# hassony2/homan

Hardware: AMD Instinct MI355X
Metric: optimisation iters/sec (30-frame 256^2 clip) (higher is better)
Workload: dtype f32

## Files before the change

### homan_amd/csrc/raster_api.hip

```cpp
#include "raster_ws.h"

RasterTune& hm_raster_tune()
{
    static thread_local RasterTune t = {0, 0, SWEEP_BLOCKS};
    return t;
}
int& hm_sweep_cap_override()
{
    static int cap = 0;
    return cap;
}

extern "C" {

size_t hm_sil_workspace_bytes(int B, int V, int F, int S)
{
    const size_t is = 2 * (size_t)S;
    size_t n = 256;
    n += al256((size_t)B * 16);
    n += al256((size_t)B * V * 3 * 4);
    n += al256((size_t)B * F * 9 * 4);
    n += al256((size_t)B * F * 8);
    n += al256((size_t)B * is * is * 4);
    n += al256((size_t)B * is * (is / 16) * 2);
    n += al256((size_t)B * S * S * 4);
    n += al256((size_t)B * (S / 8) * (S / 8) * 16);
    n += al256((size_t)B * is * is * 4);
    n += al256((size_t)B * is * (is / 16) * 4);
    n += al256((size_t)B * is * (is / 16) * 4);
    n += al256((size_t)B * F * 24 * 4);
    n += al256((size_t)B * F * 2);
    n += al256((size_t)B * SR_MAX * 8);
    n += al256((size_t)B * (S / 16) * (S / 16));
    n += al256((size_t)B * SR_MAX * F * 4);
    n += al256(4 * (size_t)B * is * (is / 64) * 16);
    n += al256((size_t)B * 2 * is * 16);
    n += al256(4 * (size_t)B * is * is * sizeof(SweepSrc));
    n += al256((size_t)B * F * sizeof(SweepFace));
    n += al256((size_t)B * F * 4) * 2;
    n += al256(sweep_ucap(B, F) * 4);
    n += al256(sweep_slot_cap(B, F) * 24);
    n += al256(ts_units(B, F, S) * 16);
    n += al256(ts_raster_units(B, S) * 4) * 3;
    return n;
}

int hm_tune_raster_lds_pad(int bytes)
{
    const int prev = hm_raster_tune().raster_lds_pad;
    if (bytes >= 0) hm_raster_tune().raster_lds_pad = bytes;
    return prev;
}
int hm_tune_raster_reorder(int enable)
{
    const int prev = hm_raster_tune().raster_reorder;
    if (enable >= 0) hm_raster_tune().raster_reorder = enable ? 1 : 0;
    return prev;
// ... 2 lines not shown
int hm_tune_sweep_blocks(int blocks)
{
    const int prev = hm_raster_tune().sweep_blocks;
    if (blocks > 0) hm_raster_tune().sweep_blocks = blocks;
    return prev;
}

int hm_sil_fwd_phase_clips(const float* verts, const int* faces, int faces_bstride, const float* K, int B, int V, int F, int S,
                           float orig_size, float znear, float zfar, const float* keep, const float* ref,
                           const float* keep_sum, float* pooled, float* loss_out, const int* work_order, float* pooled_depth,
                           float* alpha_full, int mask_shared, const float* rigid_rot6d, const float* rigid_trans,
                           const float* rigid_scale, int rigid_abs, int persistent_outputs, void* workspace, int clip_len,
                           int out_stride, float* cam_verts_out, int phases, hipStream_t stream)
{
    HM_CHECK_ARG(phases >= 1 && phases <= 3);
    HM_CHECK_ARG(verts && faces && K && pooled && workspace && HM_CLIP_LEN_OK(B, clip_len));
    if (clip_len == 0) clip_len = B;
    HM_CHECK_ARG(!rigid_rot6d || (rigid_trans && rigid_scale));
    HM_CHECK_ARG(B > 0 && V > 0 && F > 0 && S > 0);
    if (S % 16 != 0 || 2 * S > 8192 || 2L * F >= (1L << 30) || B >= 32768) return HM_ERR_UNSUPPORTED;
    HM_CHECK_ARG(faces_bstride == 0 || faces_bstride == 3 * F);
    SilWs w = carve(workspace, B, V, F, S);
    const int is = 2 * S;
    int* bins = is <= (SR_MAX == 64 ? 1024 : 0) ? w.bin_cnt : nullptr;
    HM_CHECK_ARG(!cam_verts_out || rigid_rot6d);
    if (phases & 1)
        hm_launch_setup_faces(w, verts, K, orig_size, faces, faces_bstride, B, V, F, is, bins, rigid_rot6d, rigid_trans, rigid_scale,
                              rigid_abs, clip_len, cam_verts_out, stream);
    if (!(phases & 2)) return hm_launch_status();
    const bool fused = keep && ref;
    const RasterTune& tune = hm_raster_tune();
    RasterFwdArgs a = {B, F, S, znear, zfar, pooled, keep, ref, fused, work_order, pooled_depth, bins, 1, persistent_outputs,
                       alpha_full, mask_shared, fused && (alpha_full || (mask_shared & 2)), tune.raster_reorder != 0,
                       tune.raster_lds_pad};
    hm_launch_raster_fwd(w, a, stream);
    if (fused && keep_sum && loss_out) hm_launch_sil_reduce(w, B, S, keep_sum, loss_out, nullptr, clip_len, out_stride, stream);
    return hm_launch_status();
}
int hm_sil_fwd_clips(const float* verts, const int* faces, int faces_bstride, const float* K, int B, int V, int F, int S,
                     float orig_size, float znear, float zfar, const float* keep, const float* ref,
                     const float* keep_sum, float* pooled, float* loss_out, const int* work_order, float* pooled_depth,
                     float* alpha_full, int mask_shared, const float* rigid_rot6d, const float* rigid_trans,
                     const float* rigid_scale, int rigid_abs, int persistent_outputs, void* workspace, int clip_len,
                     int out_stride, float* cam_verts_out, hipStream_t stream)
{
    return hm_sil_fwd_phase_clips(verts, faces, faces_bstride, K, B, V, F, S, orig_size, znear, zfar, keep, ref, keep_sum, pooled,
                                  loss_out, work_order, pooled_depth, alpha_full, mask_shared, rigid_rot6d, rigid_trans,
// ... 10 lines not shown
                            loss_out, work_order, pooled_depth, alpha_full, mask_shared, rigid_rot6d, rigid_trans,
                            rigid_scale, rigid_abs, persistent_outputs, workspace, 0, 0, nullptr, stream);
}

size_t hm_sil_render_bytes(void) { return sizeof(HmSilRender); }
int hm_sil_fwd_multi(const HmSilRender* renders, int n, int phases, hipStream_t stream)
{
    HM_CHECK_ARG(renders && n >= 1 && n <= HM_MAX_RENDERS && phases >= 1 && phases <= 3);
    SilWs ws[HM_MAX_RENDERS];
    SetupFacesArgs sa[HM_MAX_RENDERS];
    RasterFwdArgs ra[HM_MAX_RENDERS];
    const RasterTune& tune = hm_raster_tune();
    for (int g = 0; g < n; ++g) {
        const HmSilRender& r = renders[g];
        HM_CHECK_ARG(r.verts && r.faces && r.K && r.pooled && r.workspace && HM_CLIP_LEN_OK(r.B, r.clip_len));
        HM_CHECK_ARG(!r.rigid_rot6d || (r.rigid_trans && r.rigid_scale));
        HM_CHECK_ARG(r.B > 0 && r.V > 0 && r.F > 0 && r.S > 0 && (!r.keep == !r.ref));
        if (r.S % 16 != 0 || 2 * r.S > 8192 || 2L * r.F >= (1L << 30) || r.B >= 32768) return HM_ERR_UNSUPPORTED;
        HM_CHECK_ARG(r.faces_bstride == 0 || r.faces_bstride == 3 * r.F);
        HM_CHECK_ARG(!r.cam_verts_out || r.rigid_rot6d);
        for (int q = 0; q < g; ++q) HM_CHECK_ARG(renders[q].workspace != r.workspace);
        ws[g] = carve(r.workspace, r.B, r.V, r.F, r.S);
        const int is = 2 * r.S;
        int* bins = is <= (SR_MAX == 64 ? 1024 : 0) ? ws[g].bin_cnt : nullptr;
        const SetupFacesArgs s1 = {r.verts, r.K, r.orig_size, r.faces, r.faces_bstride, r.B, r.V, r.F, is, bins, r.rigid_rot6d,
                                   r.rigid_trans, r.rigid_scale, r.rigid_abs, r.clip_len ? r.clip_len : r.B, r.cam_verts_out};
        sa[g] = s1;
        const bool fused = r.keep && r.ref;
        const RasterFwdArgs r1 = {r.B, r.F, r.S, r.znear, r.zfar, r.pooled, r.keep, r.ref, fused, r.work_order, r.pooled_depth, bins, 1,
                                  r.persistent_outputs, nullptr, r.mask_shared & 1, false, tune.raster_reorder != 0, tune.raster_lds_pad};
        ra[g] = r1;
    }
    if (phases & 1) hm_launch_setup_faces_multi(ws, sa, n, stream);
    if (phases & 2) hm_launch_raster_fwd_multi(ws, ra, n, stream);
    return hm_launch_status();
}

int hm_sil_hint_near_winding(void* workspace, int winding, hipStream_t stream)
{
    HM_CHECK_ARG(workspace && (winding == 0 || winding == 1));
    return hipMemsetAsync((char*)workspace + 24 * 4, winding, 1, stream) == hipSuccess ? HM_OK : HM_ERR_LAUNCH;
}

int hm_sil_reduce_clips(int B, int V, int F, int S, const float* keep_sum, float* loss_out, float* frame_out,
                        void* workspace, int clip_len, int out_stride, hipStream_t stream)
{
    HM_CHECK_ARG(workspace && B > 0 && S > 0 && (frame_out || loss_out) && (!loss_out || keep_sum));
// ... 64 lines not shown
                        background, rgb, stream);
    return hm_launch_status();
}


int hm_bench_sil_kernels(const float* verts, const int* faces, const float* K, int B, int V, int F, int S,
                         const float* keep, const float* ref, const float* keep_sum, float* pooled, float* loss_out,
                         const int* work_order, const int* adj_off, const int* adj_items,
                         const float* upstream, float* grad_verts, void* workspace, int reps, float* avg_ms,
                         hipStream_t stream)
{
    HM_CHECK_ARG(verts && faces && K && keep && ref && keep_sum && pooled && loss_out && workspace && reps > 0 && avg_ms);
    HM_CHECK_ARG(adj_off && adj_items && upstream && grad_verts);
    int rc = hm_sil_fwd(verts, faces, 0, K, B, V, F, S, 1.0f, 0.1f, 100.0f, keep, ref, keep_sum, pooled, loss_out,
                        work_order, nullptr, nullptr, 0, nullptr, nullptr, nullptr, 0, 0, workspace, stream);
    if (rc != HM_OK) return rc;
    rc = hm_sil_bwd(verts, K, B, V, F, S, 1.0f, 1e-3f, 1, upstream, nullptr, keep_sum, adj_off, adj_items,
                    grad_verts, nullptr, workspace, 0, stream);
    if (rc != HM_OK) return rc;
    SilWs w = carve(workspace, B, V, F, S);
    hipEvent_t e0, e1;
    if (hipEventCreate(&e0) != hipSuccess || hipEventCreate(&e1) != hipSuccess) return HM_ERR_LAUNCH;
    float ms = 0.f;
    int* bins = 2 * S <= 1024 ? w.bin_cnt : nullptr;
    hm_launch_setup_faces(w, verts, K, 1.0f, faces, 0, B, V, F, 2 * S, bins, nullptr, nullptr, nullptr, 0, B, nullptr, stream);
    RasterFwdArgs a = {B, F, S, 0.1f, 100.0f, pooled, keep, ref, true, work_order, nullptr, bins, 0, 1, nullptr, 0, false, false, 0};
    (void)hipEventRecord(e0, stream);
    for (int i = 0; i < reps; ++i) hm_launch_raster_fwd(w, a, stream);
    (void)hipEventRecord(e1, stream);
    (void)hipEventSynchronize(e1);
    (void)hipEventElapsedTime(&ms, e0, e1);
    avg_ms[0] = ms / (float)reps;
    (void)hipMemsetAsync(w.bin_cnt, 0, (size_t)B * SR_MAX * 4, stream);
    (void)hipEventRecord(e0, stream);
    for (int i = 0; i < reps; ++i) hm_launch_sweep(w, B, F, S, 1e-3f, 0, stream);
    (void)hipEventRecord(e1, stream);
    (void)hipEventSynchronize(e1);
    (void)hipEventElapsedTime(&ms, e0, e1);
    avg_ms[1] = ms / (float)reps;
    (void)hipEventRecord(e0, stream);
    for (int i = 0; i < reps; ++i) hm_launch_lines(w, B, F, S, 1, upstream, keep_sum, B, stream);
    (void)hipEventRecord(e1, stream);
    (void)hipEventSynchronize(e1);
    (void)hipEventElapsedTime(&ms, e0, e1);
    avg_ms[2] = ms / (float)reps;
    (void)hipEventDestroy(e0);
    (void)hipEventDestroy(e1);
    return hm_launch_status();
}

size_t hm_sil_timestamps_bytes(int B, int V, int F, int S) { (void)V; return ts_units(B, F, S) * 16; }
int hm_sil_timestamps(void* workspace, int B, int V, int F, int S, int enable, hipStream_t stream)
{
    HM_CHECK_ARG(workspace && B > 0 && F > 0 && S > 0);
    SilWs w = carve(workspace, B, V, F, S);
    if (hipMemsetAsync((char*)workspace + 24 * 4 + 1, enable ? 1 : 0, 1, stream) != hipSuccess) return HM_ERR_LAUNCH;
// ... 31 lines not shown
    }
    free(t);
    return HM_OK;
}
int hm_debug_sweep_caps(int cap)
{
    const int prev = hm_sweep_cap_override();
    hm_sweep_cap_override() = cap > 0 ? cap : 0;
    return prev;
}

int hm_sil_read_idx_map(const void* workspace, int B, int V, int F, int S, int* out, hipStream_t stream)
{
    SilWs w = carve((void*)workspace, B, V, F, S);
    return hipMemcpyAsync(out, w.idx_map, (size_t)B * 4 * S * S * 4, hipMemcpyDeviceToDevice, stream) == hipSuccess
               ? HM_OK : HM_ERR_LAUNCH;
}
int hm_sil_read_boxes(const void* workspace, int B, int V, int F, int S, void* out, hipStream_t stream)
{
    SilWs w = carve((void*)workspace, B, V, F, S);
    return hipMemcpyAsync(out, w.boxes, (size_t)B * F * 8, hipMemcpyDeviceToDevice, stream) == hipSuccess ? HM_OK
                                                                                                         : HM_ERR_LAUNCH;
}
int hm_sil_read_faces9(const void* workspace, int B, int V, int F, int S, float* out, hipStream_t stream)
{
    SilWs w = carve((void*)workspace, B, V, F, S);
    return hipMemcpyAsync(out, w.faces9, (size_t)B * F * 9 * 4, hipMemcpyDeviceToDevice, stream) == hipSuccess
               ? HM_OK : HM_ERR_LAUNCH;
}
int hm_sil_invalidate_outputs(void* workspace, int B, int V, int F, int S, hipStream_t stream)
{
    HM_CHECK_ARG(workspace && B > 0 && S > 0);
    SilWs w = carve(workspace, B, V, F, S);
    return hipMemsetAsync(w.region_state, 0, (size_t)B * (S / 16) * (S / 16), stream) == hipSuccess ? HM_OK : HM_ERR_LAUNCH;
}
int hm_sil_read_parts(const void* workspace, int B, int V, int F, int S, double* out, hipStream_t stream)
{
    SilWs w = carve((void*)workspace, B, V, F, S);
    return hipMemcpyAsync(out, w.parts, (size_t)B * F * 6 * 8, hipMemcpyDeviceToDevice, stream) == hipSuccess
               ? HM_OK : HM_ERR_LAUNCH;
}
}
```

### homan_amd/csrc/raster_common.h

```cpp
#pragma once
#include "hm_common.h"
#include <type_traits>

#define HM_TILE 8
#define HM_STILE 16
#define RASTER_WAVES 4
#define STAGE_DW 20

typedef int hm_v2i __attribute__((ext_vector_type(2)));
typedef unsigned hm_v4u __attribute__((ext_vector_type(4)));
#ifndef RASTER_NT_STORES
#define RASTER_NT_STORES 0
#endif
__device__ __forceinline__ void hm_out_store(float* p, float v)
{
#if RASTER_NT_STORES
    __builtin_nontemporal_store(v, p);
#else
    *p = v;
#endif
}
__device__ __forceinline__ void hm_out_store2(int* p, int a, int b)
{
#if RASTER_NT_STORES
// ... 15 lines not shown

struct FaceBox {
    unsigned short x0m, y0, x1, y1;
};

__device__ __forceinline__ float topix(float v, int is)
{
    float a = v * (float)is;
    a = a + (float)is;
    a = a - 1.0f;
    return 0.5f * a;
}
__device__ __forceinline__ bool backside(const float* f)
{
    return (f[7] - f[1]) * (f[3] - f[0]) < (f[4] - f[1]) * (f[6] - f[0]);
}
__device__ __forceinline__ void wave_sync()
{
    __builtin_amdgcn_fence(__ATOMIC_ACQ_REL, "wavefront");
    __builtin_amdgcn_wave_barrier();
}

#define SR_MAX 64
__host__ __device__ __forceinline__ int hm_sr_shift(int is) { return is <= 512 ? 6 : 7; }

__device__ __forceinline__ int hm_wave_scan_incl(int v)
{
    v += __builtin_amdgcn_update_dpp(0, v, 0x111, 0xf, 0xf, false);
    v += __builtin_amdgcn_update_dpp(0, v, 0x112, 0xf, 0xf, false);
    v += __builtin_amdgcn_update_dpp(0, v, 0x114, 0xf, 0xf, false);
    v += __builtin_amdgcn_update_dpp(0, v, 0x118, 0xf, 0xf, false);
    v += __builtin_amdgcn_update_dpp(0, v, 0x142, 0xa, 0xf, false);
    v += __builtin_amdgcn_update_dpp(0, v, 0x143, 0xc, 0xf, false);
    return v;
}

__device__ __forceinline__ float rlane(float v, int l)
{
    return __builtin_bit_cast(float, __builtin_amdgcn_readlane(__builtin_bit_cast(int, v), l));
}

__device__ __forceinline__ unsigned spread8(unsigned x)
{
    x = (x | (x << 4)) & 0x0f0fu;
    x = (x | (x << 2)) & 0x3333u;
    x = (x | (x << 1)) & 0x5555u;
    return x;
// ... 125 lines not shown
```

### homan_amd/csrc/raster_fwd.hip

```cpp
#include "raster_ws.h"

#ifdef RASTER_TRACE
#define RASTER_TRACE_WGS 65536
__device__ unsigned g_raster_trace[RASTER_TRACE_WGS][9];
__device__ int g_raster_trace_F = 0, g_raster_trace_depth = -1;
#define RPH_MARK(k) do { if (tid == 0) { const unsigned long long t_ = wall_clock64(); rtr[k] += (unsigned)(t_ - rtr_t); rtr_t = t_; } } while (0)
#elif defined(RASTER_PHASES)
__device__ unsigned long long g_raster_ph[24];
#define RPH_MARK(k) do { if (tid == 0) { const unsigned long long t_ = clock64(); rph[k] += t_ - rph_t; rph_t = t_; } } while (0)
#else
#define RPH_MARK(k)
#endif
#ifndef CAND_CAP
#define CAND_CAP 512
#endif
#ifndef RB_PASS
#define RB_PASS 128
#endif
#ifndef HM_PRUNE
#define HM_PRUNE 1
#endif
#ifndef RASTER_WPE
#define RASTER_WPE 6
#endif
// ... 19 lines not shown
    __shared__ int wsum[RASTER_WAVES];
    __shared__ int cand_n[2];
    const int w = __builtin_amdgcn_readfirstlane((int)(threadIdx.x >> 6)), lane = threadIdx.x & 63, tid = threadIdx.x;
    const int is = 2 * S, tiles_x = S / HM_TILE, ntiles = tiles_x * tiles_x, regions_x = tiles_x / 2;
    const bool dyn = wo_dyn && hint[2] != 0u;
    const int wo = __builtin_amdgcn_readfirstlane(dyn ? wo_dyn[blk]
                                                     : work_order ? work_order[blk] : (int)(((blk % B) << 16) | (blk / B)));
    if (wo_dyn && !dyn && threadIdx.x == 0) wo_dyn[blk] = wo;
    const int region = wo & 0xffff, b = wo >> 16;
    const int rx = region % regions_x, ry = region / regions_x;
    const int tx = 2 * rx + (w & 1), ty = 2 * ry + (w >> 1);
    const int tile = ty * tiles_x + tx;

    const int gx0 = rx * 2 * HM_STILE, gx1 = gx0 + 2 * HM_STILE - 1;
    const int gy1 = is - 1 - ry * 2 * HM_STILE, gy0 = gy1 - (2 * HM_STILE - 1);
    const float gcx0 = (float)(2 * gx0 + 1 - is) / (float)is, gcx1 = (float)(2 * gx1 + 1 - is) / (float)is;
    const float gcy0 = (float)(2 * gy0 + 1 - is) / (float)is, gcy1 = (float)(2 * gy1 + 1 - is) / (float)is;
    const bool pow2 = (is & (is - 1)) == 0;
    const float inv_is = 1.0f / (float)is;
    const unsigned long long zb_empty = ((unsigned long long)__float_as_uint(zfar) << 32) | 0xffffffffull;

    int had_any = 0;
    const uint2* bx = reinterpret_cast<const uint2*>(boxes) + (long)b * F;
    const int nsx = (is + (1 << hm_sr_shift(is)) - 1) >> hm_sr_shift(is);
    const int sr = (gy0 >> hm_sr_shift(is)) * nsx + (gx0 >> hm_sr_shift(is));
    unsigned char* rstate = region_state + (long)b * regions_x * regions_x + region;
    const int nscan = bin_cnt ? bin_cnt[b * nsx * nsx + sr] : F;
    const int rstate0 = persistent ? (int)*rstate : 0;
    const int* scan = bin_cnt ? bin_list + ((long)b * nsx * nsx + sr) * F : nullptr;
    const bool idle = nscan == 0 && rstate0 == 1;
    const bool ts_on = hm_ts_enabled(hint) && tid == 0;
    if (ts_on) hm_ts_store(ts_slots, blk, 0, ts_t0);
#ifdef RASTER_TRACE
    unsigned rtr[6] = {0, 0, 0, 0, 0, 0}, rtr_cand = 0, rtr_units = 0;
    unsigned long long rtr_t = ts_t0;
#endif
#ifdef RASTER_PHASES
    unsigned long long rph[6] = {0, 0, 0, 0, 0, 0}, rph_t = clock64();
    unsigned long long rph_units[3] = {0, 0, 0};
    unsigned rph_pairs = 0;
    __shared__ unsigned s_rph_iters;
    if (tid == 0) s_rph_iters = 0u;
    __syncthreads();
#endif
    if (!idle) {
#pragma unroll
        for (int k = 0; k < 4; ++k) zb[tid + 256 * k] = zb_empty;
// ... 69 lines not shown
            const float xf = (float)(xb + c4), yf = (float)(yb + j);
            float wgt[3], ws = 0.0f;
#pragma unroll
            for (int q = 0; q < 3; ++q) {
                float t = iv[3 * q] * xf;
                t = t + iv[3 * q + 1] * yf;
                t = t + iv[3 * q + 2];
                t = fminf(fmaxf(t, 0.0f), 1.0f);
                wgt[q] = t;
                ws += t;
            }
            float sum = wgt[0] * rz0;
            sum = sum + wgt[1] * rz1;
            sum = sum + wgt[2] * rz2;
            const float zp = ws / sum;
            if (zp > znear && zp < zfar)
                atomicMin(&zb[(sy0 + j) * 32 + sx0 + c4],
                          ((unsigned long long)__float_as_uint(zp) << 32) | (unsigned)fn);
        }
    };
    for (int cbase = 0; cbase < nscan; cbase += CAND_CAP) {
        if (tid == 0) { cand_n[0] = 0; cand_n[1] = 0; }
        __syncthreads();
        uint2 v[CAND_CAP / 256];
        int vf[CAND_CAP / 256];
#pragma unroll
        for (int k = 0; k < CAND_CAP / 256; ++k) {
            const int e = cbase + k * 256 + tid;
            vf[k] = e < nscan ? (scan ? scan[e] : e) : -1;
        }
#pragma unroll
        for (int k = 0; k < CAND_CAP / 256; ++k) v[k] = vf[k] >= 0 ? bx[vf[k]] : make_uint2(0u, 0u);
#pragma unroll
        for (int k = 0; k < CAND_CAP / 256; ++k) {
            const int fi = vf[k];
            const int x0 = v[k].x & 0x3fff, y0 = (int)(v[k].x >> 16), x1 = (int)(v[k].y & 0xffff), y1 = (int)(v[k].y >> 16);
            const unsigned m = (x1 < gx0 || x0 > gx1 || y1 < gy0 || y0 > gy1) ? 0u : ((v[k].x >> 14) & 3u);
#pragma unroll
            for (int var = 0; var < 2; ++var) {
                const bool hit = (m >> var) & 1u;
                const unsigned long long bal = __ballot(hit);
                if (bal == 0ull) continue;
                const int cls = var == near_w ? 0 : 1;
                int basep = 0;
                if (lane == 0) basep = atomicAdd(&cand_n[cls], __popcll(bal));
                basep = __builtin_amdgcn_readfirstlane(basep);
                const int at = basep + __popcll(bal & ((1ull << lane) - 1ull));
                if (hit) cand[cls ? 2 * CAND_CAP - 1 - at : at] = fi | (var << 30);
            }
        }
        __syncthreads();
        RPH_MARK(0);
        had_any |= cand_n[0] | cand_n[1];
        const int n_near = cand_n[0], n_far = cand_n[1];
        for (int e0 = 0; e0 < n_near || e0 < n_far; e0 += RB_PASS / 2) {
            int units = 0;
            const int cls = tid >> 6, ci = e0 + (tid & 63);
            if (tid < RB_PASS && ci < (cls ? n_far : n_near)) {
                const int e = cand[cls ? 2 * CAND_CAP - 1 - ci : ci];
                const int fi = e & 0x3fffffff, var = e >> 30;
// ... 107 lines not shown
#ifdef RASTER_PHASES
                    if (lane == 0) atomicAdd(&g_raster_ph[21], (unsigned long long)__popcll(bal));
#endif
                    if (pass) uq[w][qn + __popcll(bal & ((1ull << lane) - 1ull))] = (unsigned short)ent;
                    qn += __popcll(bal);
                    wave_sync();
                    if (qn >= 64) {
                        qn -= 64;
                        const int e = uq[w][qn + lane];
                        wave_sync();
                        unit_body(e & 0xff, e >> 8);
                    }
                }
                if (lane < qn) {
                    const int e = uq[w][lane];
                    unit_body(e & 0xff, e >> 8);
                }
            }
            __syncthreads();
            RPH_MARK(4);
        }
    }
    __syncthreads();
    if (tid == 0 && bin_cnt && reset_bins) {
        const int per_side = (1 << hm_sr_shift(is)) / (2 * HM_STILE);
        const int rw = min(per_side, regions_x - per_side * (gx0 >> hm_sr_shift(is))), rh = min(per_side, regions_x - per_side * (gy0 >> hm_sr_shift(is)));
        const int slot = b * nsx * nsx + sr;
        if (atomicAdd(done + slot, 1u) == (unsigned)(rw * rh) - 1u) {
            bin_cnt[slot] = 0;
            atomicExch(done + slot, 0u);
        }
    }

    if (persistent && !had_any && rstate0 == 1) {
#ifdef RASTER_PHASES
        if (tid == 0) atomicAdd(&g_raster_ph[7], 1ull);
#endif
        if (wg_cost && tid == 0) wg_cost[blk] = 0u;
        return;
    }
    __syncthreads();
    if (tid == 0) *rstate = (persistent && !had_any) ? 1 : 0;

    const int r = ty * HM_TILE + (lane >> 3), c = tx * HM_TILE + (lane & 7);
    const int xi0 = 2 * c, yi0 = is - 1 - 2 * r;
    float zmin[4];
    int imin[4];
#pragma unroll
    for (int s4 = 0; s4 < 4; ++s4) {
        const int dy = s4 >> 1, dx = s4 & 1;
        const unsigned long long key = zb[(yi0 - dy - gy0) * 32 + (xi0 + dx - gx0)];
        zmin[s4] = __uint_as_float((unsigned)(key >> 32));
        imin[s4] = (int)(unsigned)(key & 0xffffffffull);
    }

    int* im = idx_map + (long)b * is * is;
#pragma unroll
    for (int dy = 0; dy < 2; ++dy) {
        hm_out_store2(im + (long)(yi0 - dy) * is + xi0, imin[2 * dy], imin[2 * dy + 1]);
    }
#pragma unroll
// ... 241 lines not shown
```

### homan_amd/csrc/raster_setup.hip

```cpp
#include "raster_ws.h"

__device__ __forceinline__ void project_vertex(const float* __restrict__ p, const float* __restrict__ k, float orig_size,
                                               float* out)
{
    const float x = ((p[0] + p[1] * 0.0f) + p[2] * 0.0f) + 0.0f;
    const float y = ((p[0] * 0.0f + p[1]) + p[2] * 0.0f) + 0.0f;
    const float z = ((p[0] * 0.0f + p[1] * 0.0f) + p[2]) + 0.0f;
    const float zz = z + 1e-9f;
    float xn = x / zz, yn = y / zz;
    {
        const float r2 = xn * xn + yn * yn;
        const float r6 = (r2 * r2) * r2;
        if (!(r6 <= 3.402823466e38f)) xn = yn = __builtin_nanf("");
    }
    float u = xn * k[0] + yn * k[1];
    u = u + k[2];
    float v = xn * k[3] + yn * k[4];
    v = v + k[5];
    v = orig_size - v;
    u = 2.0f * (u - orig_size / 2.0f) / orig_size;
    v = 2.0f * (v - orig_size / 2.0f) / orig_size;
    out[0] = u; out[1] = v; out[2] = z;
}

__device__ __forceinline__ void setup_faces_body(const int bx, const int by, const float* __restrict__ verts, const float* __restrict__ K,
                                                     float orig_size, const int* __restrict__ faces, int faces_bstride,
                                                     int B, int V, int F, int is, float* __restrict__ faces9,
                                                     FaceBox* __restrict__ boxes, unsigned char* __restrict__ owned,
                                                     int* __restrict__ bin_cnt, int* __restrict__ bin_list,
                                                     const float* __restrict__ rigid_rot6d,
                                                     const float* __restrict__ rigid_trans,
                                                     const float* __restrict__ rigid_scale, int rigid_abs, int clip_len,
                                                     float* __restrict__ cam_out, int nfb)
{
    HM_STAMP_START(0);
    __shared__ int s_cnt[SR_MAX], s_base[SR_MAX];
    __shared__ float s_R[9];
    if (rigid_rot6d && threadIdx.x == 0) rot6d_to_mat(rigid_rot6d + by * 6, s_R);
    if (bx >= nfb) {
        __syncthreads();
        const int bb = by, v = (bx - nfb) * blockDim.x + threadIdx.x;
        if (v >= V) return;
        float sc = rigid_scale[bb / clip_len];
        if (rigid_abs) sc = fabsf(sc);
        const float* m = verts + ((long)bb * V + v) * 3;
        const float x = sc * m[0], y = sc * m[1], z = sc * m[2];
        const float* t = rigid_trans + bb * 3;
        float* o = cam_out + ((long)bb * V + v) * 3;
        o[0] = x * s_R[0] + y * s_R[3] + z * s_R[6] + t[0];
        o[1] = x * s_R[1] + y * s_R[4] + z * s_R[7] + t[1];
        o[2] = x * s_R[2] + y * s_R[5] + z * s_R[8] + t[2];
        return;
    }
    const int b = by, fi = bx * blockDim.x + threadIdx.x;
    const bool valid = fi < F;
    const int nsx = (is + (1 << hm_sr_shift(is)) - 1) >> hm_sr_shift(is), nsr = nsx * nsx;
    if (threadIdx.x < SR_MAX) s_cnt[threadIdx.x] = 0;
    __syncthreads();
    unsigned mask = 0;
    int x0 = 1, y0 = 1, x1 = 0, y1 = 0;
    if (valid) {
        const long i = (long)b * F + fi;
        const int* fc = faces + (long)b * faces_bstride + 3 * fi;
        float f[9], r[9];
#pragma unroll
        for (int k = 0; k < 3; ++k) {
            const float* mv = verts + ((long)b * V + fc[k]) * 3;
            float cam[3] = {mv[0], mv[1], mv[2]};
            if (rigid_rot6d) {
                float sc = rigid_scale[b / clip_len];
                if (rigid_abs) sc = fabsf(sc);
                const float x = sc * mv[0], y = sc * mv[1], z = sc * mv[2];
                const float* t = rigid_trans + b * 3;
                cam[0] = x * s_R[0] + y * s_R[3] + z * s_R[6] + t[0];
                cam[1] = x * s_R[1] + y * s_R[4] + z * s_R[7] + t[1];
                cam[2] = x * s_R[2] + y * s_R[5] + z * s_R[8] + t[2];
            }
            project_vertex(cam, K + b * 9, orig_size, f + 3 * k);
        }
#pragma unroll
// ... 6 lines not shown
        float px[3], py[3];
#pragma unroll
        for (int k = 0; k < 3; ++k) { px[k] = topix(f[3 * k], is); py[k] = topix(f[3 * k + 1], is); }
        const float xmin = fminf(px[0], fminf(px[1], px[2])), xmax = fmaxf(px[0], fmaxf(px[1], px[2]));
        const float ymin = fminf(py[0], fminf(py[1], py[2])), ymax = fmaxf(py[0], fmaxf(py[1], py[2]));
        if (!(xmax >= -2.0f && ymax >= -2.0f && xmin <= is + 1.0f && ymin <= is + 1.0f)) mask = 0;
#pragma unroll
        for (int k = 0; k < 3; ++k)
            if (!(fabsf(f[3 * k]) <= 1e15f && fabsf(f[3 * k + 1]) <= 1e15f)) mask = 0;
        x0 = max(0, (int)ceilf(fmaxf(xmin, -2.0f) - 0.01f));
        x1 = min(is - 1, (int)floorf(fminf(xmax, is + 1.0f) + 0.01f));
        y0 = max(0, (int)ceilf(fmaxf(ymin, -2.0f) - 0.01f));
        y1 = min(is - 1, (int)floorf(fminf(ymax, is + 1.0f) + 0.01f));
        if (x1 < x0 || y1 < y0) mask = 0;
        if (mask == 0) { x0 = y0 = 1; x1 = y1 = 0; }
        FaceBox bx;
        bx.x0m = (unsigned short)(x0 | (mask << 14));
        bx.y0 = (unsigned short)y0;
        bx.x1 = (unsigned short)x1;
        bx.y1 = (unsigned short)y1;
        boxes[i] = bx;
    }
    if (!bin_cnt) return;
    const int sx0 = x0 >> hm_sr_shift(is), sx1 = x1 >> hm_sr_shift(is), sy0 = y0 >> hm_sr_shift(is), sy1 = y1 >> hm_sr_shift(is);
    int local[4];
    int nloc = 0;
    if (mask)
        for (int sy = sy0; sy <= sy1; ++sy)
            for (int sx = sx0; sx <= sx1; ++sx) {
                if (nloc < 4) local[nloc] = atomicAdd(&s_cnt[sy * nsx + sx], 1);
                ++nloc;
            }
    __syncthreads();
    if (threadIdx.x < nsr) {
        const int c = s_cnt[threadIdx.x];
        s_base[threadIdx.x] = c ? atomicAdd(&bin_cnt[b * nsr + threadIdx.x], c) : 0;
    }
    __syncthreads();
    if (mask) {
        int q = 0;
        for (int sy = sy0; sy <= sy1; ++sy)
            for (int sx = sx0; sx <= sx1; ++sx, ++q) {
                const int sr = sy * nsx + sx;
                const int at = q < 4 ? s_base[sr] + local[q] : atomicAdd(&bin_cnt[b * nsr + sr], 1);
                bin_list[((long)b * nsr + sr) * F + at] = fi;
            }
    }
    HM_STAMP_END(0);
}

__global__ __launch_bounds__(256) void k_setup_faces(SetupFacesK a)
{
    setup_faces_body((int)blockIdx.x, (int)blockIdx.y, a.verts, a.K, a.orig_size, a.faces, a.faces_bstride, a.B, a.V, a.F, a.is, a.faces9,
                     a.boxes, a.owned, a.bin_cnt, a.bin_list, a.rigid_rot6d, a.rigid_trans, a.rigid_scale, a.rigid_abs, a.clip_len,
                     a.cam_out, a.nfb);
}
__global__ __launch_bounds__(256) void k_setup_faces_multi(SetupFacesMulti m)
{
    int g = 0;
#pragma unroll
    for (int k = 1; k < HM_MAX_RENDERS; ++k) g += (k < m.n && (int)blockIdx.y >= m.first[k]) ? 1 : 0;
    g = __builtin_amdgcn_readfirstlane(g);
    const SetupFacesK& a = m.r[g];
    if ((int)blockIdx.x >= m.nblk[g]) return;
    setup_faces_body((int)blockIdx.x, (int)blockIdx.y - m.first[g], a.verts, a.K, a.orig_size, a.faces, a.faces_bstride, a.B, a.V, a.F,
                     a.is, a.faces9, a.boxes, a.owned, a.bin_cnt, a.bin_list, a.rigid_rot6d, a.rigid_trans, a.rigid_scale,
                     a.rigid_abs, a.clip_len, a.cam_out, a.nfb);
}

// ... 43 lines not shown
```

### homan_amd/csrc/raster_ws.h

```cpp
#pragma once
#include "raster_common.h"

#define HM_INTERNAL __attribute__((visibility("hidden")))

#ifndef SWEEP_BLOCKS
#define SWEEP_BLOCKS 1280
#endif
struct RasterTune {
    int raster_lds_pad;
    int raster_reorder;
    int sweep_blocks;
};
HM_INTERNAL RasterTune& hm_raster_tune();
HM_INTERNAL int& hm_sweep_cap_override();
#define TS_SWEEP_WGS 4096
static inline size_t ts_raster_units(int B, int S) { return (size_t)B * (S / 8) * (S / 8) / RASTER_WAVES; }
static inline size_t ts_lines_units(int B, int F, int S) { return (size_t)B * F / 256 + 2 * (size_t)B + 64 + (size_t)B * S / 2 + 8; }
static inline size_t ts_units(int B, int F, int S) { return ts_raster_units(B, S) + ts_lines_units(B, F, S) + 4 * TS_SWEEP_WGS; }
static inline size_t sweep_ucap(int B, int F) { return (size_t)B * F * 4 + 1024; }
static inline size_t sweep_slot_cap(int B, int F) { return sweep_ucap(B, F) + (size_t)B * F; }

static inline size_t al256(size_t x) { return (x + 255) & ~(size_t)255; }

struct SilWs {
    unsigned int* counter; float* frame_rec;
    float* ndc; float* faces9; FaceBox* boxes; int* idx_map; unsigned short* alpha16; float* dimg;
    float* partials; float* gimg; unsigned short* planes; double* parts;
    unsigned char* owned; int* bin_cnt; unsigned int* bin_done; unsigned char* region_state; int* bin_list;
    uint4* lrec; SweepSrc* srcs; unsigned short* lsum;
    SweepList sweep;
    unsigned long long* ts;
    int* wo_dyn; int* wo_tmp; unsigned int* wg_cost;
};
static inline SilWs carve(void* ws, int B, int V, int F, int S)
{
    const size_t is = 2 * (size_t)S;
    char* p = (char*)ws;
    SilWs w;
    w.counter = (unsigned int*)p; p += 256;
    w.frame_rec = (float*)p; p += al256((size_t)B * 16);
    w.ndc = (float*)p; p += al256((size_t)B * V * 3 * 4);
    w.faces9 = (float*)p; p += al256((size_t)B * F * 9 * 4);
    w.boxes = (FaceBox*)p; p += al256((size_t)B * F * 8);
    w.idx_map = (int*)p; p += al256((size_t)B * is * is * 4);
    w.alpha16 = (unsigned short*)p; p += al256((size_t)B * is * (is / 16) * 2);
    w.dimg = (float*)p; p += al256((size_t)B * S * S * 4);
    w.partials = (float*)p; p += al256((size_t)B * (S / 8) * (S / 8) * 16);
    w.gimg = (float*)p; p += al256((size_t)B * is * is * 4);
    w.planes = (unsigned short*)p; p += al256((size_t)B * is * (is / 16) * 4) * 2;
    w.parts = (double*)p; p += al256((size_t)B * F * 24 * 4);
    w.owned = (unsigned char*)p; p += al256((size_t)B * F * 2);
    w.bin_cnt = (int*)p; w.bin_done = (unsigned int*)(p + (size_t)B * SR_MAX * 4); p += al256((size_t)B * SR_MAX * 8);
    w.region_state = (unsigned char*)p; p += al256((size_t)B * (S / 16) * (S / 16));
    w.bin_list = (int*)p; p += al256((size_t)B * SR_MAX * F * 4);
    w.lrec = (uint4*)p; p += al256(4 * (size_t)B * is * (is / 64) * 16);
    w.lsum = (unsigned short*)p; p += al256((size_t)B * 2 * is * 16);
    w.srcs = (SweepSrc*)p; p += al256(4 * (size_t)B * is * is * sizeof(SweepSrc));
    w.sweep.tab = (SweepFace*)p; p += al256((size_t)B * F * sizeof(SweepFace));
    w.sweep.offs = (int*)p; p += al256((size_t)B * F * 4);
    w.sweep.tickets = (unsigned int*)p; p += al256((size_t)B * F * 4);
    w.sweep.ufirst = (unsigned int*)p; p += al256(sweep_ucap(B, F) * 4);
    w.sweep.upart = (float*)p; p += al256(sweep_slot_cap(B, F) * 24);
    w.ts = (unsigned long long*)p; p += al256(ts_units(B, F, S) * 16);
    w.wo_dyn = (int*)p; p += al256(ts_raster_units(B, S) * 4);
    w.wo_tmp = (int*)p; p += al256(ts_raster_units(B, S) * 4);
    w.wg_cost = (unsigned int*)p;
    w.sweep.cnt = (unsigned long long*)(w.counter + 16);
    w.sweep.done = w.counter + 18;
    w.sweep.total = (unsigned long long*)(w.counter + 20);
    w.sweep.ucap = (int)sweep_ucap(B, F);
    w.sweep.slot_cap = (int)sweep_slot_cap(B, F);
    if (hm_sweep_cap_override() > 0) {
        w.sweep.ucap = min(w.sweep.ucap, hm_sweep_cap_override());
        w.sweep.slot_cap = min(w.sweep.slot_cap, hm_sweep_cap_override());
    }
    return w;
}
// ... 55 lines not shown
```

### include/homan_amd.h

```cpp
#ifndef HOMAN_AMD_H
#define HOMAN_AMD_H

#include <stddef.h>

#ifdef __cplusplus
extern "C" {
#endif

#ifndef HIP_INCLUDE_HIP_HIP_RUNTIME_API_H
typedef struct ihipStream_t* hipStream_t;
#endif

#define HM_OK 0
#define HM_ERR_BAD_ARG (-1)
#define HM_ERR_LAUNCH (-2)
#define HM_ERR_UNSUPPORTED (-3)

int hm_rigid_fwd(const float* mesh, const float* rot6d, const float* trans, const float* scale, int abs_scale, int N,
                 int V, float* rotmat, float* verts, hipStream_t stream);
int hm_rigid_bwd(const float* mesh, const float* rot6d, const float* scale, int abs_scale, const float* const* g_terms,
                 const float* weights, int n_terms, const float* g_rigid, const float* g_frame, int frame_stride,
                 float frame_scale, int N, int V, float* g_mesh, float* g_rot6d, float* g_trans, float* g_scale_part,
                 void* workspace, hipStream_t stream);
size_t hm_rigid_workspace_bytes(int N);
// ... 51 lines not shown
int hm_ordinal_depth_fwd(const float* d0, const float* d1, const float* a0, const float* a1, const unsigned char* m0,
                         const unsigned char* m1, int B, int S, float* frame_part, float* rec, float* out1,
                         void* workspace, hipStream_t stream);
int hm_ordinal_depth_bwd(const float* d0, const float* d1, const float* a0, const float* a1, const unsigned char* m0,
                         const unsigned char* m1, int B, int S, const float* rec, const float* upstream, float* g0,
                         float* g1, hipStream_t stream);
int hm_ordinal_depth_bwd_flags(const float* d0, const float* d1, const float* a0, const float* a1, const unsigned char* m0,
                               const unsigned char* m1, int B, int S, const float* rec, const float* upstream, float* g0,
                               float* g1, unsigned char* flags0, unsigned char* flags1, hipStream_t stream);
int hm_tune_sweep_blocks(int blocks);
int hm_tune_raster_lds_pad(int bytes);
int hm_tune_raster_reorder(int enable);
int hm_tune_nn_lds_pad(int bytes);
int hm_debug_sweep_caps(int cap);
int hm_shade_rgb(const float* verts, const int* faces, int faces_bstride, const float* textures, int B, int V, int F, int S,
                 const float* light_dir, float intensity_ambient, float intensity_directional, const float* background,
                 float* rgb, void* workspace, hipStream_t stream);
const double* hm_sil_parts(const void* workspace, int B, int V, int F, int S);
int hm_sil_read_idx_map(const void* workspace, int B, int V, int F, int S, int* out, hipStream_t stream);
int hm_sil_read_faces9(const void* workspace, int B, int V, int F, int S, float* out, hipStream_t stream);
int hm_sil_invalidate_outputs(void* workspace, int B, int V, int F, int S, hipStream_t stream);
int hm_sil_read_parts(const void* workspace, int B, int V, int F, int S, double* out, hipStream_t stream);
int hm_sil_read_boxes(const void* workspace, int B, int V, int F, int S, void* out, hipStream_t stream);

size_t hm_softsil_workspace_bytes(int B, int V, int F, int S);
int hm_softsil_fwd(const float* verts, const int* faces, const float* K, int B, int V, int F, int S, float orig_size,
                   float znear, float zfar, const float* sigma, float* alpha, void* workspace, hipStream_t stream);
int hm_softsil_bwd(const float* verts, const int* faces, const float* K, int B, int V, int F, int S, float orig_size,
                   float znear, float zfar, const float* sigma, const float* alpha, const float* grad_alpha,
                   const int* adj_off, const int* adj_items, float* grad_verts, void* workspace, hipStream_t stream);
size_t hm_softsil_pose_workspace_bytes(int N, int S);
int hm_softsil_pose_terms(const float* alpha, const float* keep, const float* ref, int N, int S, float* terms, float* grad,
                          void* workspace, hipStream_t stream);
int hm_sigma_anneal(float* sigma, float decay, float sigma_min, hipStream_t stream);

size_t hm_reduce_workspace_bytes(void);
int hm_v2d_fwd(const float* verts, const float* camintr, int hand_nb, const float* ref2d, float image_size, int N,
               int V, float* unit_grad, float* out2, void* workspace, hipStream_t stream);
int hm_smooth_fwd(const float* verts, int N, int V, int hand_nb, float* unit_grad, float* out1, void* workspace,
                  hipStream_t stream);
int hm_priors_fwd(const float* pca, long npca, const float* s_obj, const float* m_obj, const float* s_hand,
                  const float* m_hand, float* g_pca, float* g_sobj, float* g_shand, float* out3, hipStream_t stream);
int hm_inter_fwd(const float* verts_hand, const float* verts_obj, const float* camintr, int B, int Vh, int Vo,
                 float expansion, float zthresh, float* frame_rec, float* out1, void* workspace, hipStream_t stream);
int hm_inter_bwd(const float* frame_rec, const float* upstream, int B, int Vh, int Vo, float* g_hand, float* g_obj,
                 hipStream_t stream);
// ... 172 lines not shown
```

Baseline: 6612.

## Bin faces per region with finer bins and pre-encoded coverage masks

```diff
diff --git a/homan_amd/csrc/raster_api.hip b/homan_amd/csrc/raster_api.hip
--- a/homan_amd/csrc/raster_api.hip
+++ b/homan_amd/csrc/raster_api.hip
@@ -30,9 +30,9 @@
     n += al256((size_t)B * is * (is / 16) * 4);
     n += al256((size_t)B * F * 24 * 4);
     n += al256((size_t)B * F * 2);
-    n += al256((size_t)B * SR_MAX * 8);
+    n += al256(ws_bin_counter_bytes(B, S));
     n += al256((size_t)B * (S / 16) * (S / 16));
-    n += al256((size_t)B * SR_MAX * F * 4);
+    n += al256(ws_bin_list_bytes(B, F, S));
     n += al256(4 * (size_t)B * is * (is / 64) * 16);
     n += al256((size_t)B * 2 * is * 16);
     n += al256(4 * (size_t)B * is * is * sizeof(SweepSrc));
@@ -81,7 +81,7 @@
     HM_CHECK_ARG(faces_bstride == 0 || faces_bstride == 3 * F);
     SilWs w = carve(workspace, B, V, F, S);
     const int is = 2 * S;
-    int* bins = is <= (SR_MAX == 64 ? 1024 : 0) ? w.bin_cnt : nullptr;
+    int* bins = is <= HM_BINS_MAX_IS ? w.bin_cnt : nullptr;
     HM_CHECK_ARG(!cam_verts_out || rigid_rot6d);
     if (phases & 1)
         hm_launch_setup_faces(w, verts, K, orig_size, faces, faces_bstride, B, V, F, is, bins, rigid_rot6d, rigid_trans, rigid_scale,
@@ -138,7 +138,7 @@
         for (int q = 0; q < g; ++q) HM_CHECK_ARG(renders[q].workspace != r.workspace);
         ws[g] = carve(r.workspace, r.B, r.V, r.F, r.S);
         const int is = 2 * r.S;
-        int* bins = is <= (SR_MAX == 64 ? 1024 : 0) ? ws[g].bin_cnt : nullptr;
+        int* bins = is <= HM_BINS_MAX_IS ? ws[g].bin_cnt : nullptr;
         const SetupFacesArgs s1 = {r.verts, r.K, r.orig_size, r.faces, r.faces_bstride, r.B, r.V, r.F, is, bins, r.rigid_rot6d,
                                    r.rigid_trans, r.rigid_scale, r.rigid_abs, r.clip_len ? r.clip_len : r.B, r.cam_verts_out};
         sa[g] = s1;
@@ -249,7 +249,7 @@
     hipEvent_t e0, e1;
     if (hipEventCreate(&e0) != hipSuccess || hipEventCreate(&e1) != hipSuccess) return HM_ERR_LAUNCH;
     float ms = 0.f;
-    int* bins = 2 * S <= 1024 ? w.bin_cnt : nullptr;
+    int* bins = 2 * S <= HM_BINS_MAX_IS ? w.bin_cnt : nullptr;
     hm_launch_setup_faces(w, verts, K, 1.0f, faces, 0, B, V, F, 2 * S, bins, nullptr, nullptr, nullptr, 0, B, nullptr, stream);
     RasterFwdArgs a = {B, F, S, 0.1f, 100.0f, pooled, keep, ref, true, work_order, nullptr, bins, 0, 1, nullptr, 0, false, false, 0};
     (void)hipEventRecord(e0, stream);
@@ -258,7 +258,7 @@
     (void)hipEventSynchronize(e1);
     (void)hipEventElapsedTime(&ms, e0, e1);
     avg_ms[0] = ms / (float)reps;
-    (void)hipMemsetAsync(w.bin_cnt, 0, (size_t)B * SR_MAX * 4, stream);
+    if (bins) (void)hipMemsetAsync(w.bin_cnt, 0, (size_t)B * ws_bins(S) * 4, stream);
     (void)hipEventRecord(e0, stream);
     for (int i = 0; i < reps; ++i) hm_launch_sweep(w, B, F, S, 1e-3f, 0, stream);
     (void)hipEventRecord(e1, stream);
@@ -336,6 +336,12 @@
     return hipMemcpyAsync(out, w.boxes, (size_t)B * F * 8, hipMemcpyDeviceToDevice, stream) == hipSuccess ? HM_OK
                                                                                                          : HM_ERR_LAUNCH;
 }
+int hm_sil_read_owned(const void* workspace, int B, int V, int F, int S, void* out, hipStream_t stream)
+{
+    SilWs w = carve((void*)workspace, B, V, F, S);
+    return hipMemcpyAsync(out, w.owned, (size_t)B * F * 2, hipMemcpyDeviceToDevice, stream) == hipSuccess ? HM_OK
+                                                                                                         : HM_ERR_LAUNCH;
+}
 int hm_sil_read_faces9(const void* workspace, int B, int V, int F, int S, float* out, hipStream_t stream)
 {
     SilWs w = carve((void*)workspace, B, V, F, S);
diff --git a/homan_amd/csrc/raster_common.h b/homan_amd/csrc/raster_common.h
--- a/homan_amd/csrc/raster_common.h
+++ b/homan_amd/csrc/raster_common.h
@@ -61,7 +61,15 @@
 }
 
 #define SR_MAX 64
-__host__ __device__ __forceinline__ int hm_sr_shift(int is) { return is <= 512 ? 6 : 7; }
+#define RB_MAX 256
+#define HM_BINS_MAX_IS 1024
+__host__ __device__ __forceinline__ bool hm_region_bins(int is) { return is <= 512; }
+__host__ __device__ __forceinline__ int hm_sr_shift(int is) { return hm_region_bins(is) ? 5 : 7; }
+__host__ __device__ __forceinline__ int hm_bins_per_side(int is) { return (is + (1 << hm_sr_shift(is)) - 1) >> hm_sr_shift(is); }
+__host__ __device__ __forceinline__ int hm_bins_per_frame(int is)
+{
+    return is <= HM_BINS_MAX_IS ? hm_bins_per_side(is) * hm_bins_per_side(is) : 0;
+}
 
 __device__ __forceinline__ int hm_wave_scan_incl(int v)
 {
diff --git a/homan_amd/csrc/raster_fwd.hip b/homan_amd/csrc/raster_fwd.hip
--- a/homan_amd/csrc/raster_fwd.hip
+++ b/homan_amd/csrc/raster_fwd.hip
@@ -65,7 +65,8 @@
 
     int had_any = 0;
     const uint2* bx = reinterpret_cast<const uint2*>(boxes) + (long)b * F;
-    const int nsx = (is + (1 << hm_sr_shift(is)) - 1) >> hm_sr_shift(is);
+    const bool own_bin = bin_cnt && hm_region_bins(is);
+    const int nsx = hm_bins_per_side(is);
     const int sr = (gy0 >> hm_sr_shift(is)) * nsx + (gx0 >> hm_sr_shift(is));
     unsigned char* rstate = region_state + (long)b * regions_x * regions_x + region;
     const int nscan = bin_cnt ? bin_cnt[b * nsx * nsx + sr] : F;
@@ -181,20 +182,36 @@
     for (int cbase = 0; cbase < nscan; cbase += CAND_CAP) {
         if (tid == 0) { cand_n[0] = 0; cand_n[1] = 0; }
         __syncthreads();
-        uint2 v[CAND_CAP / 256];
+        if (own_bin && reset_bins && cbase == 0 && tid == 0) bin_cnt[b * nsx * nsx + sr] = 0;
         int vf[CAND_CAP / 256];
-#pragma unroll
-        for (int k = 0; k < CAND_CAP / 256; ++k) {
-            const int e = cbase + k * 256 + tid;
-            vf[k] = e < nscan ? (scan ? scan[e] : e) : -1;
-        }
-#pragma unroll
-        for (int k = 0; k < CAND_CAP / 256; ++k) v[k] = vf[k] >= 0 ? bx[vf[k]] : make_uint2(0u, 0u);
+        unsigned vm[CAND_CAP / 256];
+        if (own_bin) {
+#pragma unroll
+            for (int k = 0; k < CAND_CAP / 256; ++k) {
+                const int e = cbase + k * 256 + tid;
+                const unsigned ent = e < nscan ? (unsigned)scan[e] : 0u;
+                vf[k] = (int)(ent & 0x3fffffffu);
+                vm[k] = ent >> 30;
+            }
+        } else {
+            uint2 v[CAND_CAP / 256];
+#pragma unroll
+            for (int k = 0; k < CAND_CAP / 256; ++k) {
+                const int e = cbase + k * 256 + tid;
+                vf[k] = e < nscan ? (scan ? scan[e] : e) : -1;
+            }
+#pragma unroll
+            for (int k = 0; k < CAND_CAP / 256; ++k) v[k] = vf[k] >= 0 ? bx[vf[k]] : make_uint2(0u, 0u);
+#pragma unroll
+            for (int k = 0; k < CAND_CAP / 256; ++k) {
+                const int x0 = v[k].x & 0x3fff, y0 = (int)(v[k].x >> 16), x1 = (int)(v[k].y & 0xffff), y1 = (int)(v[k].y >> 16);
+                vm[k] = (x1 < gx0 || x0 > gx1 || y1 < gy0 || y0 > gy1) ? 0u : ((v[k].x >> 14) & 3u);
+            }
+        }
 #pragma unroll
         for (int k = 0; k < CAND_CAP / 256; ++k) {
             const int fi = vf[k];
-            const int x0 = v[k].x & 0x3fff, y0 = (int)(v[k].x >> 16), x1 = (int)(v[k].y & 0xffff), y1 = (int)(v[k].y >> 16);
-            const unsigned m = (x1 < gx0 || x0 > gx1 || y1 < gy0 || y0 > gy1) ? 0u : ((v[k].x >> 14) & 3u);
+            const unsigned m = vm[k];
 #pragma unroll
             for (int var = 0; var < 2; ++var) {
                 const bool hit = (m >> var) & 1u;
@@ -348,7 +365,7 @@
         }
     }
     __syncthreads();
-    if (tid == 0 && bin_cnt && reset_bins) {
+    if (tid == 0 && bin_cnt && reset_bins && !own_bin) {
         const int per_side = (1 << hm_sr_shift(is)) / (2 * HM_STILE);
         const int rw = min(per_side, regions_x - per_side * (gx0 >> hm_sr_shift(is))), rh = min(per_side, regions_x - per_side * (gy0 >> hm_sr_shift(is)));
         const int slot = b * nsx * nsx + sr;
@@ -363,6 +380,14 @@
         if (tid == 0) atomicAdd(&g_raster_ph[7], 1ull);
 #endif
         if (wg_cost && tid == 0) wg_cost[blk] = 0u;
+#ifdef RASTER_TRACE
+        if (tid == 0 && nscan > 0 && blk < RASTER_TRACE_WGS && (g_raster_trace_F == 0 || g_raster_trace_F == F) &&
+            (g_raster_trace_depth < 0 || g_raster_trace_depth == (pooled_depth ? 1 : 0))) {
+            unsigned* o = g_raster_trace[blk];
+            for (int k = 0; k < 6; ++k) o[k] = rtr[k];
+            o[6] = (unsigned)ts_t0; o[7] = 0u; o[8] = 0u;
+        }
+#endif
         return;
     }
     __syncthreads();
diff --git a/homan_amd/csrc/raster_setup.hip b/homan_amd/csrc/raster_setup.hip
--- a/homan_amd/csrc/raster_setup.hip
+++ b/homan_amd/csrc/raster_setup.hip
@@ -34,7 +34,7 @@
                                                      float* __restrict__ cam_out, int nfb)
 {
     HM_STAMP_START(0);
-    __shared__ int s_cnt[SR_MAX], s_base[SR_MAX];
+    __shared__ int s_cnt[RB_MAX], s_base[RB_MAX];
     __shared__ float s_R[9];
     if (rigid_rot6d && threadIdx.x == 0) rot6d_to_mat(rigid_rot6d + by * 6, s_R);
     if (bx >= nfb) {
@@ -54,8 +54,8 @@
     }
     const int b = by, fi = bx * blockDim.x + threadIdx.x;
     const bool valid = fi < F;
-    const int nsx = (is + (1 << hm_sr_shift(is)) - 1) >> hm_sr_shift(is), nsr = nsx * nsx;
-    if (threadIdx.x < SR_MAX) s_cnt[threadIdx.x] = 0;
+    const int nsx = hm_bins_per_side(is), nsr = nsx * nsx;
+    if (threadIdx.x < RB_MAX) s_cnt[threadIdx.x] = 0;
     __syncthreads();
     unsigned mask = 0;
     int x0 = 1, y0 = 1, x1 = 0, y1 = 0;
@@ -108,29 +108,50 @@
         boxes[i] = bx;
     }
     if (!bin_cnt) return;
-    const int sx0 = x0 >> hm_sr_shift(is), sx1 = x1 >> hm_sr_shift(is), sy0 = y0 >> hm_sr_shift(is), sy1 = y1 >> hm_sr_shift(is);
-    int local[4];
-    int nloc = 0;
-    if (mask)
-        for (int sy = sy0; sy <= sy1; ++sy)
-            for (int sx = sx0; sx <= sx1; ++sx) {
-                if (nloc < 4) local[nloc] = atomicAdd(&s_cnt[sy * nsx + sx], 1);
-                ++nloc;
-            }
-    __syncthreads();
-    if (threadIdx.x < nsr) {
-        const int c = s_cnt[threadIdx.x];
-        s_base[threadIdx.x] = c ? atomicAdd(&bin_cnt[b * nsr + threadIdx.x], c) : 0;
-    }
-    __syncthreads();
-    if (mask) {
-        int q = 0;
-        for (int sy = sy0; sy <= sy1; ++sy)
-            for (int sx = sx0; sx <= sx1; ++sx, ++q) {
-                const int sr = sy * nsx + sx;
-                const int at = q < 4 ? s_base[sr] + local[q] : atomicAdd(&bin_cnt[b * nsr + sr], 1);
-                bin_list[((long)b * nsr + sr) * F + at] = fi;
-            }
+    const int sh = hm_sr_shift(is);
+    if (hm_region_bins(is)) {
+        const int cx0 = x0 >> sh, cx1 = x1 >> sh, cy0 = y0 >> sh, cy1 = y1 >> sh;
+        if (mask)
+            for (int cy = cy0; cy <= cy1; ++cy)
+                for (int cx = cx0; cx <= cx1; ++cx) atomicAdd(&s_cnt[cy * nsx + cx], 1);
+        __syncthreads();
+        if (threadIdx.x < nsr) {
+            const int c = s_cnt[threadIdx.x];
+            s_base[threadIdx.x] = c ? atomicAdd(&bin_cnt[b * nsr + threadIdx.x], c) : 0;
+        }
+        __syncthreads();
+        if (mask)
+            for (int cy = cy0; cy <= cy1; ++cy)
+                for (int cx = cx0; cx <= cx1; ++cx) {
+                    const int bin = cy * nsx + cx;
+                    const int at = atomicAdd(&s_base[bin], 1);
+                    bin_list[((long)b * nsr + bin) * F + at] = (int)((unsigned)fi | (mask << 30));
+                }
+    } else {
+        const int sx0 = x0 >> sh, sx1 = x1 >> sh, sy0 = y0 >> sh, sy1 = y1 >> sh;
+        int local[4];
+        int nloc = 0;
+        if (mask)
+            for (int sy = sy0; sy <= sy1; ++sy)
+                for (int sx = sx0; sx <= sx1; ++sx) {
+                    if (nloc < 4) local[nloc] = atomicAdd(&s_cnt[sy * nsx + sx], 1);
+                    ++nloc;
+                }
+        __syncthreads();
+        if (threadIdx.x < nsr) {
+            const int c = s_cnt[threadIdx.x];
+            s_base[threadIdx.x] = c ? atomicAdd(&bin_cnt[b * nsr + threadIdx.x], c) : 0;
+        }
+        __syncthreads();
+        if (mask) {
+            int q = 0;
+            for (int sy = sy0; sy <= sy1; ++sy)
+                for (int sx = sx0; sx <= sx1; ++sx, ++q) {
+                    const int sr = sy * nsx + sx;
+                    const int at = q < 4 ? s_base[sr] + local[q] : atomicAdd(&bin_cnt[b * nsr + sr], 1);
+                    bin_list[((long)b * nsr + sr) * F + at] = fi;
+                }
+        }
     }
     HM_STAMP_END(0);
 }
diff --git a/homan_amd/csrc/raster_ws.h b/homan_amd/csrc/raster_ws.h
--- a/homan_amd/csrc/raster_ws.h
+++ b/homan_amd/csrc/raster_ws.h
@@ -21,6 +21,9 @@
 static inline size_t sweep_slot_cap(int B, int F) { return sweep_ucap(B, F) + (size_t)B * F; }
 
 static inline size_t al256(size_t x) { return (x + 255) & ~(size_t)255; }
+static inline size_t ws_bins(int S) { return (size_t)hm_bins_per_frame(2 * S); }
+static inline size_t ws_bin_counter_bytes(int B, int S) { return (size_t)B * ws_bins(S) * (hm_region_bins(2 * S) ? 4 : 8); }
+static inline size_t ws_bin_list_bytes(int B, int F, int S) { return (size_t)B * ws_bins(S) * F * 4; }
 
 struct SilWs {
     unsigned int* counter; float* frame_rec;
@@ -50,9 +53,10 @@
     w.planes = (unsigned short*)p; p += al256((size_t)B * is * (is / 16) * 4) * 2;
     w.parts = (double*)p; p += al256((size_t)B * F * 24 * 4);
     w.owned = (unsigned char*)p; p += al256((size_t)B * F * 2);
-    w.bin_cnt = (int*)p; w.bin_done = (unsigned int*)(p + (size_t)B * SR_MAX * 4); p += al256((size_t)B * SR_MAX * 8);
+    w.bin_cnt = (int*)p; w.bin_done = hm_region_bins(2 * S) ? nullptr : (unsigned int*)(p + (size_t)B * ws_bins(S) * 4);
+    p += al256(ws_bin_counter_bytes(B, S));
     w.region_state = (unsigned char*)p; p += al256((size_t)B * (S / 16) * (S / 16));
-    w.bin_list = (int*)p; p += al256((size_t)B * SR_MAX * F * 4);
+    w.bin_list = (int*)p; p += al256(ws_bin_list_bytes(B, F, S));
     w.lrec = (uint4*)p; p += al256(4 * (size_t)B * is * (is / 64) * 16);
     w.lsum = (unsigned short*)p; p += al256((size_t)B * 2 * is * 16);
     w.srcs = (SweepSrc*)p; p += al256(4 * (size_t)B * is * is * sizeof(SweepSrc));
diff --git a/include/homan_amd.h b/include/homan_amd.h
--- a/include/homan_amd.h
+++ b/include/homan_amd.h
@@ -97,6 +97,7 @@
 int hm_sil_invalidate_outputs(void* workspace, int B, int V, int F, int S, hipStream_t stream);
 int hm_sil_read_parts(const void* workspace, int B, int V, int F, int S, double* out, hipStream_t stream);
 int hm_sil_read_boxes(const void* workspace, int B, int V, int F, int S, void* out, hipStream_t stream);
+int hm_sil_read_owned(const void* workspace, int B, int V, int F, int S, void* out, hipStream_t stream);
 
 size_t hm_softsil_workspace_bytes(int B, int V, int F, int S);
 int hm_softsil_fwd(const float* verts, const int* faces, const float* K, int B, int V, int F, int S, float orig_size,
```

New measurement: 6752 (median of 6 runs). +2.1%, better.
